# theori-io/nrsc5

Hardware: AMD Instinct MI355X
Metric: IQ MS/s demod+decoded (higher is better)
Workload: dtype exact float32 half-band (== int16 Q15) / f32 OFDM + sync / int32 Viterbi metrics

## Files before the change

nrsc5_amd/csrc/engine.hip:

```cpp
#include <array>
#include <atomic>
#include <hip/hip_runtime.h>
#include <math.h>
#include <stdio.h>
#include <stdlib.h>
#include <string.h>
#include <algorithm>
#include <chrono>
#include <deque>
#include <new>
#include <vector>
#include "nrsc5hip.h"
#include "kernels.h"

using namespace nrsc5;

static_assert(sizeof(nrsc5hip_record) == sizeof(BlockRecord), "record ABI mismatch");
static_assert(sizeof(BlockRecord) % 8 == 0, "record alignment");

static thread_local char g_err[512] = "";

static thread_local double g_seam[14];
struct SeamClock {
    int slot; std::chrono::steady_clock::time_point t0;
// ... 5 lines not shown
    for (int k = 0; k < 8; k++) { if (out) out[k] = g_seam[k]; if (reset) g_seam[k] = 0; }
}
extern "C" void nrsc5hip_debug_seam_counts(double out[6], int reset)
{
    for (int k = 0; k < 6; k++) { if (out) out[k] = g_seam[8 + k]; if (reset) g_seam[8 + k] = 0; }
}
extern "C" const char *nrsc5hip_last_error(void) { return g_err; }
namespace nrsc5 { void set_last_error(const char *msg) { snprintf(g_err, sizeof(g_err), "%s", msg); } }
#ifndef NRSC5HIP_SOURCE_SHA
#define NRSC5HIP_SOURCE_SHA "unknown"
#endif
static const char g_source_sha_marker[] = "NRSC5HIP_SOURCE_SHA=" NRSC5HIP_SOURCE_SHA;
extern "C" const char *nrsc5hip_source_sha(void) { return g_source_sha_marker + 20; }

#define HIPCHK(expr)                                                                                   \
    do {                                                                                               \
        hipError_t _e = (expr);                                                                        \
        if (_e != hipSuccess) {                                                                        \
            snprintf(g_err, sizeof(g_err), "%s failed: %s (%s:%d)", #expr, hipGetErrorString(_e), __FILE__, __LINE__); \
            return NRSC5HIP_EHIP;                                                                      \
        }                                                                                              \
    } while (0)
#define FAIL(code, ...) do { snprintf(g_err, sizeof(g_err), __VA_ARGS__); return (code); } while (0)

struct DeviceGuard {
    int prev = -1, want = -1;
    explicit DeviceGuard(int dev) : want(dev) { if (hipGetDevice(&prev) != hipSuccess) prev = -1; if (prev != want) (void)hipSetDevice(want); }
    ~DeviceGuard() { if (prev >= 0 && prev != want) (void)hipSetDevice(prev); }
};
#define ON_ENGINE_DEVICE_FAST(e) DeviceGuard _device_guard((e) ? (e)->cfg.device : 0); if (!(e)) FAIL(NRSC5HIP_EINVAL, "null engine")
#define ON_ENGINE_DEVICE(e) ON_ENGINE_DEVICE_FAST(e); do { int _rc = settle(e); if (_rc) return _rc; } while (0)
struct nrsc5hip_engine;
static int settle(nrsc5hip_engine *e);

struct nrsc5hip_engine {
    nrsc5hip_config cfg;
    DevTables tb;
    DevBuffers db;
    struct Lane {
        hipStream_t main, aux[NAUX];
        hipEvent_t ev_window[NWIN], ev_decoded[NWIN];
        bool decoded_pending[NWIN];
        int lane_parity[NAUX];
        bool thin;
        bool acq_needed;
        bool px_needed;
        unsigned long long set_sig;
        int dec_waited;
        bool prepared_by_sync;
        long long step_count;
        long long am_step_count;
        bool am_decoded_pending[NWIN];
        int *counters_dev, *counters_host;
        DevBuffers db;
    } lane;
    int naux;
    int naux_am;
    int verdict_lag;
    int am_segments, am_warm, am_runin;
    int fwd_warm;
    int mixfft_syms;
    int sync_lanes;
    int fold_report;
    int fuse_seam_prepare;
    int tb_walk;
    int fwd_segments;
    int flow_min;
    unsigned *flow_dev; size_t flow_cap;
    unsigned *flow_err;
    long long flow_bursts, flow_steps;
    hipStream_t main;
    std::vector<void *> allocs;
    std::vector<long long> wr_host, base_host;
    std::vector<int> drained;
    std::vector<int> mode_host;
    std::vector<long long> raw_host;
    std::vector<char> attached;
    static constexpr int NSTAGE = 8;
    uint8_t *stage_pin[NSTAGE], *stage_pin_dev[NSTAGE], *stage_dev2[NSTAGE]; hipEvent_t stage_ev[NSTAGE]; bool stage_busy[NSTAGE]; int stage_slot;
    unsigned *decim_ticket;
    hipStream_t ingest; hipEvent_t ev_ingest, ev_main, ev_appended;
    bool ingest_dirty;
    bool main_stepped;
    bool main_appended;
    size_t early_flush;
    int staged_stream; size_t staged_bytes; bool staged_cu8; long long staged_q15;
    StreamReport *report_host[2], *report_dev[2];
    std::vector<long long> rd_host;
    std::vector<int> fetched;
    std::vector<char> mirror_ok;
    std::vector<std::deque<BlockRecord>> pending;
    int inflight_stream;
    unsigned report_seq;
    long long inflight_rd_pred;
    bool inflight_decoded;
    unsigned inflight_seq;
    struct Ahead { bool valid; int stream; unsigned seq; bool decoded; } ahead;
    bool inflight_progress;
    bool direct_decimate;
    bool defer_wait;
    bool counters_clean;
    std::vector<char> pred_ok;
    std::vector<int> pred_samperr, pred_bc;
    std::vector<char> manual_step;
    static constexpr long long HC_OFF = 8, HC_PREFIX = 4 * HC_OFF, HC_KEEP = 16384;
    uint8_t *hc_pin, *hc_dev; size_t hc_cap;
// ... 233 lines not shown
    st.nco_re = 1.0f; st.nco_im = 0.0f; st.nco_exact = 1;
}

static void init_am_state(AmStream &am)
{
    memset(&am, 0, sizeof(am));
    am.pli = am.hppi = am.aabi = am.rdbi = -1;
    am.am_diversity_wait = 4;
    am.dec_bc = -1;
}

extern "C" int nrsc5hip_engine_create(const nrsc5hip_config *cfg, nrsc5hip_engine **out)
{
    if (!cfg || !out) FAIL(NRSC5HIP_EINVAL, "null argument");
    *out = nullptr;
    if (cfg->max_streams < 1 || cfg->q15_capacity < 2 * WIN_N || cfg->record_capacity < 64 || cfg->p1_slots < 2)
        FAIL(NRSC5HIP_EINVAL, "bad config (max_streams>=1, q15_capacity>=%d, record_capacity>=64, p1_slots>=2)", 2 * WIN_N);
    int ndev = 0;
    HIPCHK(hipGetDeviceCount(&ndev));
    if (cfg->device < 0 || cfg->device >= ndev) FAIL(NRSC5HIP_EINVAL, "device %d out of range (%d devices)", cfg->device, ndev);
    DeviceGuard guard(cfg->device);
    nrsc5hip_engine *e = new (std::nothrow) nrsc5hip_engine();
    if (!e) FAIL(NRSC5HIP_ENOMEM, "out of host memory");
    e->cfg = *cfg;
    const size_t S = cfg->max_streams;
    if (cfg->p1_async) {
        const char *q = getenv("GPU_MAX_HW_QUEUES");
        static std::atomic<bool> warned{false};
        if ((!q || atoi(q) < 8) && !warned.exchange(true)) {
            fprintf(stderr, "libnrsc5hip: warning: p1_async engine with GPU_MAX_HW_QUEUES=%s (< 8): decode streams will share hardware queues with "
                            "the block-step chain; export GPU_MAX_HW_QUEUES=8 before the HIP runtime initialises\n", q ? q : "unset (default 4)");
        }
    }
    int rc = 0;
    do {
        {
            e->naux = 1; e->naux_am = 3;
            e->verdict_lag = 0; e->fwd_segments = 0; e->fwd_warm = 2; e->mixfft_syms = 1; e->sync_lanes = 0; e->flow_min = 0; e->tb_walk = 1; e->fuse_seam_prepare = 1; e->fold_report = 1;
            e->am_segments = 4; e->am_warm = K9_WARM; e->am_runin = K9_TB_RUNIN;
        }
        {
            nrsc5hip_engine::Lane &ln = e->lane;
            if (hipStreamCreate(&ln.main) != hipSuccess) rc = NRSC5HIP_EHIP;
            for (int k = 0; k < NAUX && !rc; k++) if (hipStreamCreate(&ln.aux[k]) != hipSuccess) rc = NRSC5HIP_EHIP;
            for (int k = 0; k < NWIN && !rc; k++) {
                if (hipEventCreate(&ln.ev_window[k]) != hipSuccess || hipEventCreate(&ln.ev_decoded[k]) != hipSuccess) rc = NRSC5HIP_EHIP;
                ln.decoded_pending[k] = false;
            }
            ln.acq_needed = true; ln.px_needed = true; ln.set_sig = 0; ln.step_count = 0; ln.am_step_count = 0;
            for (int k = 0; k < NAUX; k++) ln.lane_parity[k] = -1;
            ln.thin = false;
            for (int k = 0; k < NWIN; k++) ln.am_decoded_pending[k] = false;
            if (!rc && hipHostMalloc((void **)&ln.counters_host, 4 * sizeof(int), hipHostMallocDefault) != hipSuccess) rc = NRSC5HIP_ENOMEM;
        }
        if (rc) { snprintf(g_err, sizeof(g_err), "stream/event creation failed"); break; }
        e->main = e->lane.main;
        if (hipStreamCreate(&e->dec_stream) != hipSuccess) { rc = NRSC5HIP_EHIP; snprintf(g_err, sizeof(g_err), "hipStreamCreate failed"); break; }
        e->dec_chunk = 0; e->chunk_nbytes_dev = nullptr; e->chunk_cap = 0;
        if ((rc = build_tables(e))) break;
        DevBuffers &db = e->db;
        db.q15_cap = cfg->q15_capacity; db.p1_slots = cfg->p1_slots; db.rec_cap = cfg->record_capacity;
        if ((rc = dev_alloc(e, &db.state, S))) break;
        db.ckpt = nullptr;
        if (cfg->p1_async && cfg->l2_feedback) {
            if (cfg->record_capacity < 2 * NWIN * 16) { rc = NRSC5HIP_EINVAL; snprintf(g_err, sizeof(g_err), "p1_async with l2_feedback needs record_capacity >= %d (speculated blocks keep their records)", 2 * NWIN * 16); break; }
            if ((rc = dev_alloc(e, &db.ckpt, S * NWIN))) break;
        }
        if ((rc = dev_alloc(e, &db.q15, S * (size_t)db.q15_cap))) break;
        db.acq_win = nullptr;
        if ((cfg->batch_zero_copy || !cfg->p1_async) && (rc = dev_alloc(e, &db.acq_win, S * WIN_N))) break;
        if ((rc = dev_alloc(e, &db.acq_filt, S * WIN_N))) break;
        if ((rc = dev_alloc(e, &db.acq_list, S + 1))) break;
        if ((rc = dev_alloc(e, &db.acq_sums, S * SYM_N))) break;
        if ((rc = dev_alloc(e, &db.bins, S * NSYM * LIVE_N))) break;
        if ((rc = dev_alloc(e, &db.nco_tab, S * NSYM * SYM_N))) break;
        if ((rc = dev_alloc(e, &db.cfo_snap, S * LIVE_N * (PM_PART + 1)))) break;
        if ((rc = dev_alloc(e, &db.cfo_phase, S * NSYM * LIVE_N))) break;
        e->flow_cap = flow_words((int)S); e->flow_bursts = e->flow_steps = 0;
        if ((rc = dev_alloc(e, &e->flow_dev, e->flow_cap))) break;
        if (hipHostMalloc((void **)&e->flow_err, 2 * sizeof(unsigned), hipHostMallocDefault) != hipSuccess) { rc = NRSC5HIP_ENOMEM; break; }
        e->flow_err[0] = e->flow_err[1] = 0;
        db.loop_exact = 1;
        db.nco_policy = NCO_EXACT_FIRST_BLOCK;
        if ((rc = dev_alloc(e, &db.pm, S * NPM * PM_FRAME))) break;
        db.nstreams_alloc = (int)S;
        if ((rc = dev_alloc(e, &db.coded, (size_t)(cfg->p1_async ? NAUX : 1) * S * P1_LEN))) break;
        if ((rc = dev_alloc(e, &db.dec, (size_t)(cfg->p1_async ? NAUX : 1) * S * (size_t)(2 * (P1_LEN + 64))))) break;
        if ((rc = dev_alloc(e, &db.tbmap, (size_t)(cfg->p1_async ? NAUX : 1) * S * (size_t)(P1_LEN / 64 + 1) * 64))) break;
        if ((rc = dev_alloc(e, &db.fwd_meta, (size_t)(cfg->p1_async ? NAUX : 1) * S * (size_t)(VIT3_GMAX * VIT3_META)))) break;
        if ((rc = dev_alloc(e, &db.fwd_stats, 4))) break;
        if (hipMemset(db.fwd_stats, 0, 4 * sizeof(int)) != hipSuccess) { rc = NRSC5HIP_EHIP; break; }
        db.tb_stats = db.fwd_stats + 2;
        if ((rc = dev_alloc(e, &db.am_k9stats, 4))) break;
        if (hipMemset(db.am_k9stats, 0, 4 * sizeof(unsigned)) != hipSuccess) { rc = NRSC5HIP_EHIP; break; }
        if ((rc = dev_alloc(e, &db.pids_stage, S * NWIN * 16 * 3 * PIDS_LEN))) break;
        if ((rc = dev_alloc(e, &db.pids_rec, S * NWIN * 16))) break;
        if (hipMemset(db.pids_rec, 0xff, S * NWIN * 16 * sizeof(int)) != hipSuccess) { rc = NRSC5HIP_EHIP; break; }
        if ((rc = dev_alloc(e, &db.p1_ring, S * db.p1_slots * P1_WORDS))) break;
        db.p1_mirror = nullptr;
        if ((rc = dev_alloc(e, &db.records, S * db.rec_cap))) break;
        if ((rc = dev_alloc(e, &db.counters, 4))) break;
        {
            const size_t nax = cfg->p1_async ? NAUX : 1;
            db.px_slots = 8 * cfg->p1_slots;
            if ((rc = dev_alloc(e, &db.px_mem, S * 2 * PX_MEM))) break;
            if ((rc = dev_alloc(e, &db.px_pair, S * 4 * PX_MAX))) break;
// ... 89 lines not shown
        }
        e->hb_hist_host.assign(S, std::array<c16, 14>{});
        e->stage_slot = 0; e->staged_stream = -1; e->staged_bytes = 0; e->staged_q15 = 0; e->staged_cu8 = false;
        if ((rc = dev_alloc(e, &e->ids_dev, S))) break;
        if ((rc = dev_alloc(e, &e->nbytes_dev, S))) break;
        if ((rc = dev_alloc(e, &e->all_ids_dev, S))) break;
        std::vector<StreamState> init(S);
        std::vector<int> ident(S);
        for (size_t s = 0; s < S; s++) { init_state(init[s]); ident[s] = (int)s; }
        if (hipMemcpy(db.state, init.data(), S * sizeof(StreamState), hipMemcpyHostToDevice) != hipSuccess ||
            hipMemcpy(e->all_ids_dev, ident.data(), S * sizeof(int), hipMemcpyHostToDevice) != hipSuccess ||
            hipMemset(db.records, 0, S * db.rec_cap * sizeof(BlockRecord)) != hipSuccess ||
            hipMemset(db.pm, 0, S * NPM * PM_FRAME) != hipSuccess) { rc = NRSC5HIP_EHIP; snprintf(g_err, sizeof(g_err), "state init copy failed"); break; }
        e->wr_host.assign(S, 0); e->base_host.assign(S, 0); e->drained.assign(S, 0);
        e->mode_host.assign(S, MODE_FM); e->raw_host.assign(S, 0); e->attached.assign(S, 0);
        e->rd_host.assign(S, 0); e->fetched.assign(S, 0); e->mirror_ok.assign(S, cfg->p1_async ? 0 : 1); e->pending.assign(S, {});
        e->pred_ok.assign(S, 0); e->pred_samperr.assign(S, 0); e->pred_bc.assign(S, 0); e->manual_step.assign(S, 0);
        e->inflight_stream = -1; e->report_seq = 0; e->inflight_rd_pred = -1; e->inflight_decoded = true; e->inflight_progress = false; e->inflight_seq = 0; e->ahead.valid = false;
        e->defer_wait = true; e->direct_decimate = true; e->counters_clean = false;
        e->lane.db = db; e->lane.counters_dev = db.counters;
        e->prof_on = false; e->prof_only = -1;
        for (int k = 0; k < NRSC5HIP_PROF_CLASSES; k++) { e->prof_ms[k] = 0; e->prof_launches[k] = 0; }
    } while (0);
    if (rc) { nrsc5hip_engine_destroy(e); return rc; }
    *out = e;
    return NRSC5HIP_OK;
}

extern "C" void nrsc5hip_engine_destroy(nrsc5hip_engine *e)
{
    if (!e) return;
    DeviceGuard guard(e->cfg.device);
    (void)hipDeviceSynchronize();
    vit_scratch_free(e->vit_scratch);
    for (void *p : e->allocs) (void)hipFree(p);
    for (hipEvent_t ev : e->dec_events) (void)hipEventDestroy(ev);
    if (e->dec_stream) (void)hipStreamDestroy(e->dec_stream);
    if (e->flow_err) (void)hipHostFree(e->flow_err);
    if (e->rec_host) (void)hipHostFree(e->rec_host);
    if (e->frames_host) (void)hipHostFree(e->frames_host);
    if (e->nblocks_host) (void)hipHostFree(e->nblocks_host);
    for (int k = 0; k < nrsc5hip_engine::NSTAGE; k++) { if (e->stage_pin[k]) (void)hipHostFree(e->stage_pin[k]); if (e->stage_ev[k]) (void)hipEventDestroy(e->stage_ev[k]); }
    for (int k = 0; k < 2; k++) if (e->report_host[k]) (void)hipHostFree(e->report_host[k]);
    if (e->hc_pin) (void)hipHostFree(e->hc_pin);
    if (e->ingest) (void)hipStreamDestroy(e->ingest);
    if (e->ev_ingest) (void)hipEventDestroy(e->ev_ingest);
    if (e->ev_main) (void)hipEventDestroy(e->ev_main);
    if (e->ev_appended) (void)hipEventDestroy(e->ev_appended);
    for (auto &sp : e->prof_spans) { (void)hipEventDestroy(sp.a); (void)hipEventDestroy(sp.b); }
    for (hipEvent_t ev : e->prof_pool) (void)hipEventDestroy(ev);
    {
        nrsc5hip_engine::Lane &ln = e->lane;
        if (ln.counters_host) (void)hipHostFree(ln.counters_host);
        for (int k = 0; k < NWIN; k++) { if (ln.ev_window[k]) (void)hipEventDestroy(ln.ev_window[k]); if (ln.ev_decoded[k]) (void)hipEventDestroy(ln.ev_decoded[k]); }
        if (ln.main) (void)hipStreamDestroy(ln.main);
        for (int k = 0; k < NAUX; k++) if (ln.aux[k]) (void)hipStreamDestroy(ln.aux[k]);
    }
    delete e;
}

extern "C" void *nrsc5hip_engine_hip_stream(nrsc5hip_engine *e) { return e ? (void *)e->main : nullptr; }

static int check_stream(nrsc5hip_engine *e, int s)
{
    if (!e) FAIL(NRSC5HIP_EINVAL, "null engine");
    if (s < 0 || s >= e->cfg.max_streams) FAIL(NRSC5HIP_EINVAL, "stream %d out of range", s);
    return 0;
}

static int pick_decode_lane(nrsc5hip_engine *e, nrsc5hip_engine::Lane &ln, long long window)
{
    const int lane = (int)(window % e->naux);
    auto busy = [&](int k) { return ln.lane_parity[k] >= 0 && hipEventQuery(ln.ev_decoded[ln.lane_parity[k]]) == hipErrorNotReady; };
    if (ln.thin && busy(lane))
        for (int k = e->naux; k < NAUX; k++) if (!busy(k)) return k;
    return lane;
}

static int fwd_segments_for(const nrsc5hip_engine *e, const nrsc5hip_engine::Lane &ln, int n)
{
    if (e->fwd_segments > 0) return e->fwd_segments;
    if (ln.thin) return 16;
    const int g = 1024 / (n > 0 ? n : 1);
    return g < 1 ? 1 : g > VIT3_GMAX ? VIT3_GMAX : g;
}

static int launch_window_decode(nrsc5hip_engine *e, nrsc5hip_engine::Lane &ln, int n, const int *ids_dev, int parity, int lane)
{
    hipStream_t ax = ln.aux[lane];
    HIPCHK(hipEventRecord(ln.ev_window[parity], ln.main));
    HIPCHK(hipStreamWaitEvent(ax, ln.ev_window[parity], 0));
    { ProfScope p(e, NRSC5HIP_PROF_PIDS, ax); launch_pids_decode(e->tb, ln.db, n, ids_dev, parity, 16, ax); }
    if (ln.px_needed) { ProfScope p(e, NRSC5HIP_PROF_PIDS, ax); launch_px_decode(e->tb, ln.db, n, ids_dev, parity, lane, ax); }
    { ProfScope p(e, NRSC5HIP_PROF_P1_DEINT, ax); launch_p1_deint(e->tb, ln.db, n, ids_dev, parity, lane, ax); }
    { ProfScope p(e, NRSC5HIP_PROF_P1_VITERBI, ax); launch_p1_forward(e->tb, ln.db, n, ids_dev, parity, lane, ax, fwd_segments_for(e, ln, n), e->fwd_warm); }
    { ProfScope p(e, NRSC5HIP_PROF_P1_TRACEBACK, ax); launch_p1_traceback(e->tb, ln.db, n, ids_dev, parity, lane, ax, e->cfg.l2_feedback ? 2 : 0, fwd_segments_for(e, ln, n), e->tb_walk); }
    HIPCHK(hipEventRecord(ln.ev_decoded[parity], ax));
    ln.decoded_pending[parity] = true;
    ln.lane_parity[lane] = parity;
    return 0;
}

static int launch_inorder_p1(nrsc5hip_engine *e, nrsc5hip_engine::Lane &ln, int n, const int *ids_dev)
{
    { ProfScope p(e, NRSC5HIP_PROF_P1_DEINT, ln.main); launch_p1_deint(e->tb, ln.db, n, ids_dev, 0, 0, ln.main); }
    { ProfScope p(e, NRSC5HIP_PROF_P1_VITERBI, ln.main); launch_p1_forward(e->tb, ln.db, n, ids_dev, 0, 0, ln.main, fwd_segments_for(e, ln, n), e->fwd_warm); }
// ... 24 lines not shown
    if (ln.db.nco_tab && (ln.acq_needed || ln.db.nco_policy == NCO_EXACT_ALWAYS)) { ProfScope p(e, NRSC5HIP_PROF_PREPARE, ln.main); launch_nco_exact(ln.db, n, ids_dev, ln.main); }
    { ProfScope p(e, NRSC5HIP_PROF_MIXFFT, ln.main); launch_mixfft(e->tb, ln.db, n, ids_dev, ln.main, e->mixfft_syms, fused_prepare ? 1 : 0); }
    const int slot = async ? (int)(ln.step_count % 16) : 0;
    const int fuse = (async && !ln.acq_needed) ? 1 : 0;
    const bool fold = rep && n == 1 && !async && !ln.px_needed && !decode_pids && !decode_p1 && e->sync_lanes != 256;
    { ProfScope p(e, NRSC5HIP_PROF_SYNC, ln.main); launch_sync(e->tb, ln.db, n, ids_dev, parity, slot, fuse, (int)window, ln.main, e->sync_lanes, decode_pids ? 0 : 1, fused_prepare ? 1 : 0, ln.px_needed ? 1 : 0,
                                                                fold ? rep->out : nullptr, fold ? rep->seq : 0u, fold ? rep->first_rec : 0); }
    if (rep) rep->folded = fold;
    ln.prepared_by_sync = fuse != 0;
    if (ln.px_needed) { ProfScope p(e, NRSC5HIP_PROF_PIDS, ln.main); launch_px_deint(e->tb, ln.db, n, ids_dev, parity, slot, ln.main); }
    if (!async) {
        if (decode_pids) { ProfScope p(e, NRSC5HIP_PROF_PIDS, ln.main); launch_pids_decode(e->tb, ln.db, n, ids_dev, parity, 1, ln.main); }
        if (ln.px_needed) { ProfScope p(e, NRSC5HIP_PROF_PIDS, ln.main); launch_px_decode(e->tb, ln.db, n, ids_dev, parity, 0, ln.main); }
        if (decode_p1) { int rc = launch_inorder_p1(e, ln, n, ids_dev); if (rc) return rc; }
    } else if ((ln.step_count % 16) == 15) {
        int rc = launch_window_decode(e, ln, n, ids_dev, parity, pick_decode_lane(e, ln, window)); if (rc) return rc;
    }
    ln.step_count++;
    HIPCHK(hipGetLastError());
    return 0;
}

static int issue_flow_burst(nrsc5hip_engine *e, nrsc5hip_engine::Lane &ln, int n, const int *ids_dev, int K)
{
    const long long window = ln.step_count / 16;
    const int parity = (int)(window % NWIN), slot0 = (int)(ln.step_count % 16);
    if (slot0 + K > 16) FAIL(NRSC5HIP_EINVAL, "a dataflow burst does not cross a window boundary");
    if (slot0 == 0 && ln.decoded_pending[parity]) {
        HIPCHK(hipStreamWaitEvent(ln.main, ln.ev_decoded[parity], 0));
        ln.decoded_pending[parity] = false;
    }
    HIPCHK(hipMemsetAsync(e->flow_dev, 0, flow_words(n) * sizeof(unsigned), ln.main));
    { ProfScope p(e, NRSC5HIP_PROF_FLOW, ln.main); launch_flow(e->tb, ln.db, n, ids_dev, K, e->flow_dev, e->flow_err, parity, slot0, (int)window, ln.main); }
    ln.step_count += K;
    e->flow_bursts++; e->flow_steps += K;
    if ((ln.step_count % 16) == 0) { int rc = launch_window_decode(e, ln, n, ids_dev, parity, pick_decode_lane(e, ln, window)); if (rc) return rc; }
    HIPCHK(hipGetLastError());
    return 0;
}

static int flush_p1(nrsc5hip_engine *e, nrsc5hip_engine::Lane &ln, int n, const int *ids_dev)
{
    if (!e->cfg.p1_async) return 0;
    if (ln.step_count % 16) {
        const long long window = ln.step_count / 16;
        int rc = launch_window_decode(e, ln, n, ids_dev, (int)(window % NWIN), pick_decode_lane(e, ln, window)); if (rc) return rc;
        ln.step_count += 16 - (ln.step_count % 16);
    }
    for (int k = 0; k < NAUX; k++) HIPCHK(hipStreamSynchronize(ln.aux[k]));
    for (int k = 0; k < NWIN; k++) ln.decoded_pending[k] = false;
    return 0;
}

static int run_steps(nrsc5hip_engine *e, int n, const int *ids_dev, unsigned long long set_sig, int max_steps, int check_every, int *steps_done)
{
    nrsc5hip_engine::Lane &ln = e->lane;
    if (set_sig != ln.set_sig) { ln.acq_needed = true; ln.px_needed = true; ln.set_sig = set_sig; }
    ln.prepared_by_sync = false;
    const bool replay = e->db.ckpt != nullptr;
    int done = 0;
    for (;;) {
        bool live = n > 0;
        while (live && done < max_steps) {
            HIPCHK(hipMemsetAsync(ln.counters_dev, 0, 4 * sizeof(int), ln.main));
            int every = check_every;
            if (check_every == 16) {
                const int to_boundary = 16 - (int)(ln.step_count % 16);
                every = ln.acq_needed ? std::min(4, to_boundary) : to_boundary;
            }
            int burst = 0;
            const bool flow = e->flow_min > 0 && n >= e->flow_min && check_every == 16 && e->cfg.p1_async && e->cfg.batch_zero_copy && !ln.acq_needed && !ln.px_needed
                              && ln.prepared_by_sync && !e->dec_chunk && ln.db.nco_policy != NCO_EXACT_ALWAYS && !ln.db.sync_phase_cycles && done + every <= max_steps && every >= 2;
            if (flow) { int rc = issue_flow_burst(e, ln, n, ids_dev, every); if (rc) return rc; burst = every; }
            for (; burst < every && done + burst < max_steps; burst++) { int rc = issue_step(e, ln, n, ids_dev); if (rc) return rc; }
            if (replay && (ln.step_count % 16) == 0) {
                const long long window = ln.step_count / 16;
                const int parity = (int)(window % NWIN);
                if (ln.decoded_pending[parity]) { HIPCHK(hipStreamWaitEvent(ln.main, ln.ev_decoded[parity], 0)); ln.decoded_pending[parity] = false; }
                ProfScope p(e, NRSC5HIP_PROF_PREPARE, ln.main);
                launch_rollback(ln.db, n, ids_dev, (int)window, e->verdict_lag, ln.main);
            }
            HIPCHK(hipMemcpyAsync(ln.counters_host, ln.counters_dev, 4 * sizeof(int), hipMemcpyDeviceToHost, ln.main));
            HIPCHK(hipStreamSynchronize(ln.main));
            if (flow && (e->flow_err[0] || e->flow_err[1]))
                FAIL(NRSC5HIP_EHIP, "dataflow burst: a hand-off was never seen (symbol item of stream position %d, block step of %d): the burst's results are void", (int)e->flow_err[0] - 1, (int)e->flow_err[1] - 1);
            ln.acq_needed = ln.counters_host[1] > 0;
            ln.thin = ln.counters_host[0] * 4 < burst * n;
            ln.px_needed = ln.counters_host[2] > 0;
            if (ln.counters_host[0] == 0) live = false;
            else done += burst;
        }
        if (e->dec_chunk) { HIPCHK(hipStreamSynchronize(e->dec_stream)); e->dec_chunk = 0; }
        { int rc = flush_p1(e, ln, n, ids_dev); if (rc) return rc; }
        if (!replay) break;
        HIPCHK(hipMemsetAsync(ln.counters_dev, 0, 4 * sizeof(int), ln.main));
        launch_rollback(ln.db, n, ids_dev, (int)(ln.step_count / 16), 0, ln.main);
        HIPCHK(hipMemcpyAsync(ln.counters_host, ln.counters_dev, 4 * sizeof(int), hipMemcpyDeviceToHost, ln.main));
        HIPCHK(hipStreamSynchronize(ln.main));
        if (ln.counters_host[3] == 0) break;
        ln.acq_needed = true; ln.prepared_by_sync = false;
        if (done >= max_steps) break;
    }
    HIPCHK(hipStreamSynchronize(ln.main));
    if (e->prof_on) prof_collect(e);
    if (steps_done) *steps_done = done;
    return 0;
}

static unsigned long long set_signature(int n, const int *ids)
{
    unsigned long long h = 0xcbf29ce484222325ull ^ (unsigned long long)n;
    if (ids) for (int k = 0; k < n; k++) h = (h ^ (unsigned long long)(unsigned)ids[k]) * 0x100000001b3ull;
    return h | 1ull;
}

static int am_flush(nrsc5hip_engine *e, nrsc5hip_engine::Lane &ln, int n, const int *ids_dev)
{
    if (!e->cfg.p1_async) return 0;
    if (ln.am_step_count % 8) {
        const long long window = ln.am_step_count / 8;
        const int parity = (int)(window % NWIN), lane = (int)(window % e->naux_am);
        hipStream_t ax = ln.aux[lane];
        HIPCHK(hipEventRecord(ln.ev_window[parity], ln.main));
        HIPCHK(hipStreamWaitEvent(ax, ln.ev_window[parity], 0));
        { ProfScope p(e, NRSC5HIP_PROF_AM_DECODE, ax); launch_am_decode(e->tb, ln.db, n, ids_dev, parity, lane, e->cfg.l2_feedback, ax, e->am_segments, e->am_warm, e->am_runin); }
        ln.am_step_count += 8 - (ln.am_step_count % 8);
    }
    for (int k = 0; k < NAUX; k++) HIPCHK(hipStreamSynchronize(ln.aux[k]));
    for (int k = 0; k < NWIN; k++) ln.am_decoded_pending[k] = false;
    return 0;
}

static int run_steps_am(nrsc5hip_engine *e, int n, const int *ids_dev, int max_steps, int check_every, int *steps_done)
{
    nrsc5hip_engine::Lane &ln = e->lane;
    const bool pipe = e->cfg.p1_async != 0;
    const bool replay = ln.db.am_ckpt != nullptr;
    int done = 0;
    for (;;) {
        bool live = n > 0;
        while (live && done < max_steps) {
            HIPCHK(hipMemsetAsync(ln.counters_dev, 0, 4 * sizeof(int), ln.main));
            int burst = 0;
            for (; burst < check_every && done + burst < max_steps; burst++) {
                const long long window = ln.am_step_count / 8;
                const int parity = pipe ? (int)(window % NWIN) : -1, lane = (int)(window % e->naux_am);
                if (pipe && (ln.am_step_count % 8) == 0) {
                    if (ln.am_decoded_pending[parity]) { HIPCHK(hipStreamWaitEvent(ln.main, ln.ev_decoded[parity], 0)); ln.am_decoded_pending[parity] = false; }
                    if (replay && ln.am_step_count > 0) launch_rollback_am(ln.db, n, ids_dev, (int)window, e->verdict_lag, ln.main);
                }
                { ProfScope p(e, NRSC5HIP_PROF_AM, ln.main); launch_am_step(e->tb, ln.db, n, ids_dev, ln.main, e->cfg.l2_feedback, parity, (int)(ln.am_step_count % 8), (int)window); }
                if (pipe && (ln.am_step_count % 8) == 7) {
                    hipStream_t ax = ln.aux[lane];
                    HIPCHK(hipEventRecord(ln.ev_window[parity], ln.main));
                    HIPCHK(hipStreamWaitEvent(ax, ln.ev_window[parity], 0));
                    { ProfScope p(e, NRSC5HIP_PROF_AM_DECODE, ax); launch_am_decode(e->tb, ln.db, n, ids_dev, parity, lane, e->cfg.l2_feedback, ax, e->am_segments, e->am_warm, e->am_runin); }
// ... 1562 lines not shown
```

nrsc5_amd/csrc/k_replay.hip:

```cpp
#include <hip/hip_runtime.h>
#include "kernels.h"

namespace nrsc5 {

__device__ inline int stream_of(const int *ids, int idx) { return ids ? ids[idx] : idx; }

__global__ __launch_bounds__(256) void k_rollback(DevBuffers db, const int *ids, int cur_window, int min_age)
{
    const int s = stream_of(ids, blockIdx.x);
    StreamState &st = db.state[s];
    BlockRecord *ring = db.records + (size_t)s * db.rec_cap;
    __shared__ int sh_p;
    const int tid = threadIdx.x;
    if (tid == 0) {
        int best = -1, best_rec = 0x7fffffff;
        for (int p = 0; p < NWIN; p++) {
            const int v = st.p1_verdict[p];
            if (v == 0 || cur_window - st.p1_window[p] < min_age) continue;
            st.p1_verdict[p] = 0;
            if (v != 2) continue;
            const int a = st.p1_recabs[p];
            if (ring[a % db.rec_cap].flags & REC_DISCARDED) continue;
            if (a < best_rec) { best_rec = a; best = p; }
        }
// ... 27 lines not shown
    }
}

__global__ __launch_bounds__(256) void k_rollback_am(DevBuffers db, const int *ids, int cur_window, int min_age)
{
    const int s = stream_of(ids, blockIdx.x);
    StreamState &st = db.state[s];
    AmStream &am = db.am[s];
    BlockRecord *ring = db.records + (size_t)s * db.rec_cap;
    __shared__ int sh_p, sh_j, sh_best;
    const int tid = threadIdx.x;
    if (tid == 0) { sh_best = 0x7fffffff; sh_p = -1; sh_j = 0; }
    __syncthreads();
    int mine = 0x7fffffff;
    if (tid < NWIN * 8) {
        const int p = tid >> 3, j = tid & 7;
        AmJob &job = db.am_job[(size_t)s * NWIN + p];
        if (cur_window - job.window >= min_age
            && job.verdict[j] == 2 && job.deliver_abs[j] >= 0) {
            job.verdict[j] = 3;
            const int a = job.deliver_abs[j];
            if (!(ring[a % db.rec_cap].flags & REC_DISCARDED)) { mine = a; atomicMin(&sh_best, a); }
        }
    }
    __syncthreads();
    if (tid < NWIN * 8 && mine != 0x7fffffff && mine == sh_best) { sh_p = tid >> 3; sh_j = tid & 7; }
    __syncthreads();
    const int p = sh_p, j = sh_j;
    if (p < 0) return;
    const AmCkpt &ck = db.am_ckpt[((size_t)s * NWIN + p) * 8 + j];
    const int a = db.am_job[(size_t)s * NWIN + p].deliver_abs[j], n = st.nblocks;
    for (int r = a + 1 + tid; r < n; r += 256) atomicOr(&ring[r % db.rec_cap].flags, (uint32_t)REC_DISCARDED);
    if (tid < 31) { st.fir_hist[tid] = ck.st.fir_hist[tid]; st.stale.fir[MODE_AM][tid] = ck.st.stale.fir[MODE_AM][tid]; }
    if (tid == 0) {
        st.rd = ck.st.rd;
        st.prev_angle = ck.st.prev_angle; st.theta = ck.st.theta; st.keep_extra = ck.st.keep_extra; st.cfo = ck.st.cfo;
        st.psmi = ck.st.psmi; st.cfo_wait = ck.st.cfo_wait; st.bc = ck.st.bc; st.samperr = ck.st.samperr; st.angle = ck.st.angle;
        st.fine_epoch = ck.st.fine_epoch;
        st.stale.fir_pushed[MODE_AM] = ck.st.stale.fir_pushed[MODE_AM];
        am.pli = ck.am.pli; am.hppi = ck.am.hppi; am.aabi = ck.am.aabi; am.rdbi = ck.am.rdbi; am.offset_history = ck.am.offset_history;
        am.am_errors = ck.am.am_errors; am.am_diversity_wait = ck.am.am_diversity_wait;
        am.q_head = j == 7 ? (ck.am.q_head + 1) % 3 : ck.am.q_head;
        am.frame_slot = ck.am.frame_slot; am.vit_parity = ck.am.vit_parity; am.next_job = ck.am.next_job;
        am.dec_bc = -1;
        st.sync_state = SYNC_NONE;
        BlockRecord &rec = ring[a % db.rec_cap];
        if (rec.state_after == SYNC_FINE) { rec.state_after = SYNC_NONE; rec.flags |= REC_LOST_SYNC; }
        st.ndiscard += n - a - 1;
        atomicAdd(&db.counters[3], 1);
        atomicAdd(&db.counters[0], 1);
    }
}

void launch_rollback_am(const DevBuffers &db, int nstreams, const int *stream_ids, int cur_window, int min_age, hipStream_t st)
{
    hipLaunchKernelGGL(k_rollback_am, dim3(nstreams), dim3(256), 0, st, db, stream_ids, cur_window, min_age);
}

void launch_rollback(const DevBuffers &db, int nstreams, const int *stream_ids, int cur_window, int min_age, hipStream_t st)
{
    hipLaunchKernelGGL(k_rollback, dim3(nstreams), dim3(256), 0, st, db, stream_ids, cur_window, min_age);
}

}
```

nrsc5_amd/csrc/kernels.h:

```cpp
#pragma once
#include "nrsc5hip.h"
#include "nrsc5_dev.h"

namespace nrsc5 {

struct DevTables {
    const uint16_t *deint_lut;
    const uint16_t *pids_gather;
    const uint32_t *eq_cell;
    const uint16_t *eq_out;
    const uint32_t *scr_p1;
    const uint32_t *scr_pids;
    const float2 *twiddle;
    const float2 *twiddle_a;
    const float *shape;
    const int16_t *hb_q15;
    const int16_t *acq_q15;
    const uint32_t *px_delay_wide;
    const uint32_t *px_delay_narrow;
    const uint32_t *am_deint_p1;
    const uint32_t *am_deint_p3_ma3;
    const uint32_t *am_deint_p3_ma1;
    const int16_t *am_acq_q15;
    const float *am_shape;
// ... 29 lines not shown
    uint32_t *p1_mirror;
    int p1_slots;
    BlockRecord *records;
    int rec_cap;
    int *counters;
    long long *sync_phase_cycles;
    int8_t *px_mem;
    int8_t *px_pair;
    int8_t *px_stage;
    PxJob *px_job;
    unsigned long long *px_dec;
    uint32_t *px_ring;
    int px_slots;
    AmStream *am;
    uint8_t *am_sym;
    uint8_t *am_q;
    int8_t *am_vit;
    int am_nvit;
    unsigned long long *am_dec;
    K9Meta *am_k9meta;
    unsigned *am_k9stats;
    AmJob *am_job;
    AmCkpt *am_ckpt;
    float *am_ber;
    int8_t *am_pids_stage;
    int *am_pids_rec;
    nrsc5hip_l2_frame *l2_ring;
    nrsc5hip_l2_frame *l2_px_ring;
    nrsc5hip_l2_frame *l2_am_ring;
};

struct StreamReport { int counters[4]; long long rd; int nblocks; int nrec; BlockRecord rec[4]; unsigned seq; unsigned pad; };
void launch_decimate_fm_cu8_stream(const DevTables &tb, const DevBuffers &db, int s, const uint8_t *iq, unsigned nbytes, unsigned *ticket, hipStream_t st);
void launch_stream_tail(const DevTables &tb, const DevBuffers &db, int s, int first_rec, StreamReport *out, unsigned seq, int do_pids, hipStream_t st);

void launch_decimate_fm_cu8(const DevTables &tb, const DevBuffers &db, int nstreams, const int *stream_ids,
                            const uint8_t *iq_base, long long iq_stride, const unsigned *nbytes, unsigned max_nbytes,
                            hipStream_t st);
void launch_attach_raw(const DevBuffers &db, int nstreams, const int *stream_ids, const uint8_t *iq_base, long long iq_stride,
                       const unsigned *nbytes, hipStream_t st);
void launch_append_cs16(const DevBuffers &db, int nstreams, const int *stream_ids,
                        const int16_t *iq_base, long long iq_stride, const unsigned *nsamples, unsigned max_n, hipStream_t st);

void launch_acquire(const DevTables &tb, const DevBuffers &db, int nstreams, const int *stream_ids, hipStream_t st);
void launch_prepare(const DevBuffers &db, int nstreams, const int *stream_ids, int acq_on, hipStream_t st);
void launch_nco_exact(const DevBuffers &db, int nstreams, const int *stream_ids, hipStream_t st);
void launch_mixfft(const DevTables &tb, const DevBuffers &db, int nstreams, const int *stream_ids, hipStream_t st, int syms_per_wg = 1, int local_prepare = 0);
size_t flow_words(int n);
void launch_flow(const DevTables &tb, const DevBuffers &db, int nstreams, const int *stream_ids, int K, unsigned *flow, unsigned *err_host, int parity, int slot0, int window, hipStream_t st);
void launch_sync(const DevTables &tb, const DevBuffers &db, int nstreams, const int *stream_ids, int parity, int slot, int fuse_prepare, int window, hipStream_t st, int lanes = 0, int pids_inline = 0, int do_prepare = 0, int ext_refs = 1,
                 StreamReport *report = nullptr, unsigned report_seq = 0, int report_first = 0);
void launch_rollback(const DevBuffers &db, int nstreams, const int *stream_ids, int cur_window, int min_age, hipStream_t st);
void launch_rollback_am(const DevBuffers &db, int nstreams, const int *stream_ids, int cur_window, int min_age, hipStream_t st);
void launch_pids_decode(const DevTables &tb, const DevBuffers &db, int nstreams, const int *stream_ids, int parity, int nslots, hipStream_t st);
void launch_px_deint(const DevTables &tb, const DevBuffers &db, int nstreams, const int *stream_ids, int parity, int slot, hipStream_t st);
void launch_px_decode(const DevTables &tb, const DevBuffers &db, int nstreams, const int *stream_ids, int parity, int lane_id, hipStream_t st);
void launch_p1_deint(const DevTables &tb, const DevBuffers &db, int nstreams, const int *stream_ids, int parity, int lane_id, hipStream_t st);
void launch_p1_forward(const DevTables &tb, const DevBuffers &db, int nstreams, const int *stream_ids, int parity, int lane_id, hipStream_t st, int segments, int warm = 2);
void launch_p1_traceback(const DevTables &tb, const DevBuffers &db, int nstreams, const int *stream_ids, int parity, int lane_id, hipStream_t st, int l2_mode = 0, int parts = 4, int walk = 1);

void launch_am_decimate_cu8(const DevTables &tb, const DevBuffers &db, int nstreams, const int *stream_ids,
                            const uint8_t *iq_base, long long iq_stride, const unsigned *nbytes, unsigned max_nbytes, hipStream_t st);
void launch_am_step(const DevTables &tb, const DevBuffers &db, int nstreams, const int *stream_ids, hipStream_t st, int l2_feedback = 0, int pipeline_parity = -1, int slot = 0,
                    int window = 0);
constexpr unsigned AMT_DELAYED = 1u << 18, AMT_PUNCT = 1u << 19;
void launch_am_decode(const DevTables &tb, const DevBuffers &db, int nstreams, const int *stream_ids, int parity, int lane_id, int l2_feedback, hipStream_t st,
                      int segments, int warm, int runin);
void launch_stage_first_header(const uint32_t *words, int nwords, int nframes, int am, int threads, int *ok, hipStream_t st);
void launch_viterbi_k9_frames(const int8_t *coded, int len, int nframes, unsigned g0, unsigned g1, unsigned g2,
                              unsigned long long *dec, uint32_t *out, hipStream_t st, int phases = 3,
                              K9Meta *meta = nullptr, int segments = 1, int warm = K9_WARM, int runin = K9_TB_RUNIN, unsigned *stats = nullptr);

constexpr int L2_MAX_BYTES = 18269;
struct L2Job { const uint32_t *words; int nbits; int pad; };
void launch_l2_index(const L2Job *jobs, int njobs, nrsc5hip_l2_frame *frames, uint8_t *bytes_out, long long stride, hipStream_t st);
void launch_l2_index_window(const DevBuffers &db, int nstreams, const int *stream_ids, int parity, hipStream_t st);
void launch_l2_index_px_window(const DevBuffers &db, int nstreams, const int *stream_ids, int parity, hipStream_t st);
void launch_l2_index_am_window(const DevBuffers &db, int nstreams, const int *stream_ids, int parity, hipStream_t st);
void launch_l2_index_am_step(const DevBuffers &db, int nstreams, const int *stream_ids, hipStream_t st);

struct VitScratch { int *endlane = nullptr; int cap = 0; uint8_t *gmap = nullptr; size_t gcap = 0; int *soft = nullptr; size_t scap = 0; int *meta = nullptr; int mcap = 0; };
void vit_scratch_free(VitScratch &sc);
int launch_viterbi_frames(VitScratch &sc, const int8_t *coded, int len, int nframes, unsigned long long *dec, uint32_t *out, hipStream_t st, int phases = 3, int segments = 1, int *stats = nullptr, int warm = 2);
void launch_selftest(int *fail_count, hipStream_t st);
void launch_fft2048(const DevTables &tb, const float2 *in, float2 *out, int nffts, hipStream_t st, int form = 1);

}
```

Before: 249,400.

## Pipeline step bursts with mapped-memory counter publish instead of per-burst sync

```diff
diff --git a/nrsc5_amd/csrc/engine.hip b/nrsc5_amd/csrc/engine.hip
--- a/nrsc5_amd/csrc/engine.hip
+++ b/nrsc5_amd/csrc/engine.hip
@@ -81,6 +81,8 @@
         long long am_step_count;
         bool am_decoded_pending[NWIN];
         int *counters_dev, *counters_host;
+        BurstWord *burst_host, *burst_dev;
+        unsigned burst_seq;
         DevBuffers db;
     } lane;
     int naux;
@@ -420,6 +422,11 @@
             ln.thin = false;
             for (int k = 0; k < NWIN; k++) ln.am_decoded_pending[k] = false;
             if (!rc && hipHostMalloc((void **)&ln.counters_host, 4 * sizeof(int), hipHostMallocDefault) != hipSuccess) rc = NRSC5HIP_ENOMEM;
+            if (!rc) {
+                void *dp = nullptr;
+                if (hipHostMalloc((void **)&ln.burst_host, 2 * sizeof(BurstWord), hipHostMallocMapped) != hipSuccess || hipHostGetDevicePointer(&dp, ln.burst_host, 0) != hipSuccess) rc = NRSC5HIP_ENOMEM;
+                else { memset(ln.burst_host, 0, 2 * sizeof(BurstWord)); ln.burst_dev = (BurstWord *)dp; ln.burst_seq = 0; }
+            }
         }
         if (rc) { snprintf(g_err, sizeof(g_err), "stream/event creation failed"); break; }
         e->main = e->lane.main;
@@ -615,6 +622,7 @@
     {
         nrsc5hip_engine::Lane &ln = e->lane;
         if (ln.counters_host) (void)hipHostFree(ln.counters_host);
+        if (ln.burst_host) (void)hipHostFree(ln.burst_host);
         for (int k = 0; k < NWIN; k++) { if (ln.ev_window[k]) (void)hipEventDestroy(ln.ev_window[k]); if (ln.ev_decoded[k]) (void)hipEventDestroy(ln.ev_decoded[k]); }
         if (ln.main) (void)hipStreamDestroy(ln.main);
         for (int k = 0; k < NAUX; k++) if (ln.aux[k]) (void)hipStreamDestroy(ln.aux[k]);
@@ -745,6 +753,36 @@
     return 0;
 }
 
+struct BurstTicket { int steps; bool flow, rewinds; unsigned seq; };
+
+static int publish_burst(nrsc5hip_engine::Lane &ln, unsigned *seq)
+{
+    ln.burst_seq++;
+    if (ln.burst_seq == 0) ln.burst_seq = 2;
+    launch_burst_publish(ln.db, &ln.burst_dev[ln.burst_seq & 1], ln.burst_seq, ln.main);
+    HIPCHK(hipGetLastError());
+    *seq = ln.burst_seq;
+    return 0;
+}
+
+static int wait_burst(nrsc5hip_engine::Lane &ln, unsigned seq, const int **counters)
+{
+    const BurstWord *w = &ln.burst_host[seq & 1];
+    const volatile unsigned *p = &w->seq;
+    const auto t0 = std::chrono::steady_clock::now();
+    for (int spins = 0; __atomic_load_n(p, __ATOMIC_ACQUIRE) != seq; spins++) {
+#if defined(__x86_64__) || defined(__i386__)
+        __builtin_ia32_pause();
+#endif
+        if ((spins & 1023) == 1023 && std::chrono::steady_clock::now() - t0 > std::chrono::milliseconds(50)) {
+            HIPCHK(hipStreamSynchronize(ln.main));
+            if (__atomic_load_n(p, __ATOMIC_ACQUIRE) != seq) FAIL(NRSC5HIP_EHIP, "burst word %u never arrived (have %u)", seq, *p);
+        }
+    }
+    *counters = w->counters;
+    return 0;
+}
+
 static int run_steps(nrsc5hip_engine *e, int n, const int *ids_dev, unsigned long long set_sig, int max_steps, int check_every, int *steps_done)
 {
     nrsc5hip_engine::Lane &ln = e->lane;
@@ -752,49 +790,66 @@
     ln.prepared_by_sync = false;
     const bool replay = e->db.ckpt != nullptr;
     int done = 0;
+    HIPCHK(hipMemsetAsync(ln.counters_dev, 0, 4 * sizeof(int), ln.main));
     for (;;) {
         bool live = n > 0;
-        while (live && done < max_steps) {
-            HIPCHK(hipMemsetAsync(ln.counters_dev, 0, 4 * sizeof(int), ln.main));
-            int every = check_every;
-            if (check_every == 16) {
-                const int to_boundary = 16 - (int)(ln.step_count % 16);
-                every = ln.acq_needed ? std::min(4, to_boundary) : to_boundary;
+        int enq = done;
+        BurstTicket pend{}; bool have_pend = false;
+        auto take = [&](const BurstTicket &b) -> int {
+            const int *c = nullptr;
+            { int rc = wait_burst(ln, b.seq, &c); if (rc) return rc; }
+            if (b.flow && (e->flow_err[0] || e->flow_err[1]))
+                FAIL(NRSC5HIP_EHIP, "dataflow burst: a hand-off was never seen (symbol item of stream position %d, block step of %d): the burst's results are void", (int)e->flow_err[0] - 1, (int)e->flow_err[1] - 1);
+            ln.acq_needed = c[1] > 0;
+            ln.thin = c[0] * 4 < b.steps * n;
+            ln.px_needed = c[2] > 0;
+            if (c[0] == 0) { live = false; enq -= b.steps; }
+            else { live = true; done += b.steps; }
+            return 0;
+        };
+        for (;;) {
+            BurstTicket cur{}; bool have_cur = false;
+            if (live && enq < max_steps) {
+                int every = check_every;
+                if (check_every == 16) {
+                    const int to_boundary = 16 - (int)(ln.step_count % 16);
+                    every = ln.acq_needed ? std::min(2, to_boundary) : to_boundary;
+                }
+                int burst = 0;
+                const bool flow = e->flow_min > 0 && n >= e->flow_min && check_every == 16 && e->cfg.p1_async && e->cfg.batch_zero_copy && !ln.acq_needed && !ln.px_needed
+                                  && ln.prepared_by_sync && !e->dec_chunk && ln.db.nco_policy != NCO_EXACT_ALWAYS && !ln.db.sync_phase_cycles && enq + every <= max_steps && every >= 2;
+                if (flow) { int rc = issue_flow_burst(e, ln, n, ids_dev, every); if (rc) return rc; burst = every; }
+                for (; burst < every && enq + burst < max_steps; burst++) { int rc = issue_step(e, ln, n, ids_dev); if (rc) return rc; }
+                if (replay && (ln.step_count % 16) == 0) {
+                    const long long window = ln.step_count / 16;
+                    const int parity = (int)(window % NWIN);
+                    if (ln.decoded_pending[parity]) { HIPCHK(hipStreamWaitEvent(ln.main, ln.ev_decoded[parity], 0)); ln.decoded_pending[parity] = false; }
+                    ProfScope p(e, NRSC5HIP_PROF_PREPARE, ln.main);
+                    launch_rollback(ln.db, n, ids_dev, (int)window, e->verdict_lag, ln.main);
+                    cur.rewinds = true;
+                }
+                cur.steps = burst; cur.flow = flow;
+                { int rc = publish_burst(ln, &cur.seq); if (rc) return rc; }
+                enq += burst; have_cur = true;
             }
-            int burst = 0;
-            const bool flow = e->flow_min > 0 && n >= e->flow_min && check_every == 16 && e->cfg.p1_async && e->cfg.batch_zero_copy && !ln.acq_needed && !ln.px_needed
-                              && ln.prepared_by_sync && !e->dec_chunk && ln.db.nco_policy != NCO_EXACT_ALWAYS && !ln.db.sync_phase_cycles && done + every <= max_steps && every >= 2;
-            if (flow) { int rc = issue_flow_burst(e, ln, n, ids_dev, every); if (rc) return rc; burst = every; }
-            for (; burst < every && done + burst < max_steps; burst++) { int rc = issue_step(e, ln, n, ids_dev); if (rc) return rc; }
-            if (replay && (ln.step_count % 16) == 0) {
-                const long long window = ln.step_count / 16;
-                const int parity = (int)(window % NWIN);
-                if (ln.decoded_pending[parity]) { HIPCHK(hipStreamWaitEvent(ln.main, ln.ev_decoded[parity], 0)); ln.decoded_pending[parity] = false; }
-                ProfScope p(e, NRSC5HIP_PROF_PREPARE, ln.main);
-                launch_rollback(ln.db, n, ids_dev, (int)window, e->verdict_lag, ln.main);
-            }
-            HIPCHK(hipMemcpyAsync(ln.counters_host, ln.counters_dev, 4 * sizeof(int), hipMemcpyDeviceToHost, ln.main));
-            HIPCHK(hipStreamSynchronize(ln.main));
-            if (flow && (e->flow_err[0] || e->flow_err[1]))
-                FAIL(NRSC5HIP_EHIP, "dataflow burst: a hand-off was never seen (symbol item of stream position %d, block step of %d): the burst's results are void", (int)e->flow_err[0] - 1, (int)e->flow_err[1] - 1);
-            ln.acq_needed = ln.counters_host[1] > 0;
-            ln.thin = ln.counters_host[0] * 4 < burst * n;
-            ln.px_needed = ln.counters_host[2] > 0;
-            if (ln.counters_host[0] == 0) live = false;
-            else done += burst;
+            if (have_pend) { int rc = take(pend); if (rc) return rc; }
+            if (have_cur && cur.rewinds) { int rc = take(cur); if (rc) return rc; have_cur = false; }
+            pend = cur; have_pend = have_cur;
+            if (!have_pend && !(live && enq < max_steps)) break;
         }
         if (e->dec_chunk) { HIPCHK(hipStreamSynchronize(e->dec_stream)); e->dec_chunk = 0; }
         { int rc = flush_p1(e, ln, n, ids_dev); if (rc) return rc; }
         if (!replay) break;
-        HIPCHK(hipMemsetAsync(ln.counters_dev, 0, 4 * sizeof(int), ln.main));
+        unsigned seq = 0; const int *c = nullptr;
         launch_rollback(ln.db, n, ids_dev, (int)(ln.step_count / 16), 0, ln.main);
-        HIPCHK(hipMemcpyAsync(ln.counters_host, ln.counters_dev, 4 * sizeof(int), hipMemcpyDeviceToHost, ln.main));
-        HIPCHK(hipStreamSynchronize(ln.main));
-        if (ln.counters_host[3] == 0) break;
+        { int rc = publish_burst(ln, &seq); if (rc) return rc; }
+        { int rc = wait_burst(ln, seq, &c); if (rc) return rc; }
+        if (c[3] == 0) break;
         ln.acq_needed = true; ln.prepared_by_sync = false;
         if (done >= max_steps) break;
     }
     HIPCHK(hipStreamSynchronize(ln.main));
+    HIPCHK(hipGetLastError());
     if (e->prof_on) prof_collect(e);
     if (steps_done) *steps_done = done;
     return 0;
diff --git a/nrsc5_amd/csrc/k_replay.hip b/nrsc5_amd/csrc/k_replay.hip
--- a/nrsc5_amd/csrc/k_replay.hip
+++ b/nrsc5_amd/csrc/k_replay.hip
@@ -103,6 +103,20 @@
     }
 }
 
+__global__ __launch_bounds__(64) void k_burst_publish(int *counters, BurstWord *out, unsigned seq)
+{
+    const int t = threadIdx.x;
+    if (t < 4) { out->counters[t] = counters[t]; counters[t] = 0; }
+    __threadfence_system();
+    __syncthreads();
+    if (t == 0) *(volatile unsigned *)&out->seq = seq;
+}
+
+void launch_burst_publish(const DevBuffers &db, BurstWord *out, unsigned seq, hipStream_t st)
+{
+    hipLaunchKernelGGL(k_burst_publish, dim3(1), dim3(64), 0, st, db.counters, out, seq);
+}
+
 void launch_rollback_am(const DevBuffers &db, int nstreams, const int *stream_ids, int cur_window, int min_age, hipStream_t st)
 {
     hipLaunchKernelGGL(k_rollback_am, dim3(nstreams), dim3(256), 0, st, db, stream_ids, cur_window, min_age);
diff --git a/nrsc5_amd/csrc/kernels.h b/nrsc5_amd/csrc/kernels.h
--- a/nrsc5_amd/csrc/kernels.h
+++ b/nrsc5_amd/csrc/kernels.h
@@ -105,6 +105,8 @@
                  StreamReport *report = nullptr, unsigned report_seq = 0, int report_first = 0);
 void launch_rollback(const DevBuffers &db, int nstreams, const int *stream_ids, int cur_window, int min_age, hipStream_t st);
 void launch_rollback_am(const DevBuffers &db, int nstreams, const int *stream_ids, int cur_window, int min_age, hipStream_t st);
+struct BurstWord { int counters[4]; unsigned seq; unsigned pad[3]; };
+void launch_burst_publish(const DevBuffers &db, BurstWord *out, unsigned seq, hipStream_t st);
 void launch_pids_decode(const DevTables &tb, const DevBuffers &db, int nstreams, const int *stream_ids, int parity, int nslots, hipStream_t st);
 void launch_px_deint(const DevTables &tb, const DevBuffers &db, int nstreams, const int *stream_ids, int parity, int slot, hipStream_t st);
 void launch_px_decode(const DevTables &tb, const DevBuffers &db, int nstreams, const int *stream_ids, int parity, int lane_id, hipStream_t st);
```

Measured after the change: 252,600 (median of 3 runs). No clear change (+1.3%).
